# yuhuishi-convect/mojo-bm25

Hardware: AMD Instinct MI355X
Metric: queries/sec + achieved HBM GB/s, 10M-doc CSC index, batch=1024, k=100 (higher is better)
Workload: dtype f32; 1 GPU; c3: 10M docs / 200k vocab, batch=1024, k=100, 8 terms per query; segments=dense, n_docs=10000000, n_terms=200000, nnz=639994696, batch=1024, terms_per_query=8, k=100, tile_docs=2048, parallelism=doc-shard x1, term_lanes=8

## Files before the change

mojo-bm25_amd/csrc/bm25mi_kernels.hip:

```cpp
#include "bm25mi_internal.h"

#include <map>
#include <mutex>
#include <cstdio>
#include <cstdlib>
#include <vector>

namespace bm25mi {

enum Phase { kAll = 0, kSample = 1, kRest = 2 };

constexpr int kJ = 8;
constexpr int kWaves = 4;
constexpr int kGroup = 64;

struct IndexArgs {
  const int64_t* indptr;
  const uint32_t* rel;
  const uint16_t* ldoc;
  const float* val;
  int64_t V, ntiles, n_docs, nnz;
  int64_t doc_offset;
  int32_t nonneg;
  int32_t sparse;
// ... 481 lines not shown
        ++pos;
      }
    }
  }
  zero_acc<S>(acc);
}

template <int S>
__device__ __forceinline__ void emit_rest_slot(float* acc, int64_t tile, int64_t n_docs,
                                               uint64_t theta, uint64_t* __restrict__ slot,
                                               int32_t Cb, int32_t* __restrict__ slot_n,
                                               uint64_t* __restrict__ ovf,
                                               int32_t* __restrict__ ovf_cnt, int32_t Co) {
  constexpr int D = 1 << S;
  float4* a4 = reinterpret_cast<float4*>(acc);
  const uint32_t lane = lane_id();
  const float th = key_score((uint32_t)(theta >> 32));
  const int64_t base = tile << S;
  const int lim = (int)max<int64_t>(-1, min<int64_t>(D, n_docs - base));
  const int tie = (int)max<int64_t>(
      -1, min<int64_t>(D, (int64_t)(0xFFFFFFFFu - (uint32_t)theta) - base + 1));
  int32_t n = 0;
#pragma unroll 1
  for (int j0 = 0; j0 < D / 256; j0 += 2) {
    const float4 f0 = a4[j0 * 64 + lane], f1 = a4[(j0 + 1) * 64 + lane];
    const float fe[8] = {f0.x, f0.y, f0.z, f0.w, f1.x, f1.y, f1.z, f1.w};
    const float mx = fmaxf(fmaxf(fmaxf(fe[0], fe[1]), fmaxf(fe[2], fe[3])),
                           fmaxf(fmaxf(fe[4], fe[5]), fmaxf(fe[6], fe[7])));
    int c = 0;
    if (!(mx < th && lim == D)) {
#pragma unroll
      for (int e = 0; e < 8; ++e) {
        const int d = (int)entry_doc(4 * j0 + e, lane);
        c += (d < lim) & ((fe[e] > th) | ((fe[e] == th) & (d < tie)));
      }
    }
    if (__ballot(c > 0) == 0) continue;
    const uint32_t incl = wave_incl_scan((uint32_t)c);
    const int32_t tot = (int32_t)__builtin_amdgcn_readlane(incl, 63);
    int pos = n + (int)incl - c;
    const int32_t past = max(n, Cb);
    int obase = 0;
    if (n + tot > past) {
      if (lane == 0) obase = atomicAdd(ovf_cnt, n + tot - past);
      obase = __shfl(obase, 0, 64) - past;
    }
#pragma unroll
    for (int e = 0; e < 8; ++e) {
      const int d = (int)entry_doc(4 * j0 + e, lane);
      const bool pass = (d < lim) & ((fe[e] > th) | ((fe[e] == th) & (d < tie)));
      if (pass) {
        const uint64_t key = ((uint64_t)score_key(fe[e]) << 32) |
                             (uint64_t)(0xFFFFFFFFu - (uint32_t)(base + d));
        if (pos < Cb) slot[pos] = key;
        else if (obase + pos < Co) ovf[obase + pos] = key;
        ++pos;
      }
    }
    n += tot;
  }
  if (n > 0 && lane == 0) *slot_n = n;
  zero_acc<S>(acc);
}

constexpr int kCrossCap = 256;
template <int S>
__device__ __forceinline__ void emit_cross(float* acc, const uint16_t* xl, int32_t nx,
                                           int64_t tile, int64_t n_docs, uint64_t theta,
                                           uint64_t* __restrict__ slot, int32_t Cb,
                                           int32_t* __restrict__ slot_n,
                                           uint64_t* __restrict__ ovf,
                                           int32_t* __restrict__ ovf_cnt, int32_t Co) {
  constexpr int D = 1 << S;
  const uint32_t lane = lane_id();
  const float th = key_score((uint32_t)(theta >> 32));
  const int64_t base = tile << S;
  const int lim = (int)max<int64_t>(-1, min<int64_t>(D, n_docs - base));
  const int tie = (int)max<int64_t>(
      -1, min<int64_t>(D, (int64_t)(0xFFFFFFFFu - (uint32_t)theta) - base + 1));
  int32_t n = 0;
  for (int32_t i0 = 0; i0 < nx; i0 += 64) {
    const int32_t i = i0 + (int32_t)lane;
    const uint32_t off = i < nx ? (uint32_t)xl[i] : 0u;
    const int d = (int)(off >> 2);
    const float f = i < nx ? atomicExch(&acc[d], -1.0f) : -1.0f;
    const bool pass = i < nx && f >= 0.f && d < lim && ((f > th) | ((f == th) & (d < tie)));
    const uint64_t m = __ballot(pass);
    if (m == 0ull) continue;
    const int32_t tot = (int32_t)__popcll(m);
    const int pos = n + (int)__builtin_amdgcn_mbcnt_hi((uint32_t)(m >> 32),
                                                     __builtin_amdgcn_mbcnt_lo((uint32_t)m, 0u));
    const int32_t past = max(n, Cb);
    int obase = 0;
    if (n + tot > past) {
      if (lane == 0) obase = atomicAdd(ovf_cnt, n + tot - past);
      obase = __shfl(obase, 0, 64) - past;
    }
    if (pass) {
      const uint64_t key = ((uint64_t)score_key(f) << 32) |
                           (uint64_t)(0xFFFFFFFFu - (uint32_t)(base + d));
      if (pos < Cb) slot[pos] = key;
      else if (obase + pos < Co) ovf[obase + pos] = key;
    }
    n += tot;
  }
  if (n > 0 && lane == 0) *slot_n = n;
  zero_acc<S>(acc);
}

template <int PH>
__device__ __forceinline__ int64_t tile_of(int64_t ti, int P, int G) {
  return PH == kSample ? sample_tile(ti, P, G) : ti;
}
template <int PH>
__device__ __forceinline__ int32_t tile_of32(uint32_t ti, uint32_t P, uint32_t G) {
  return (int32_t)(PH == kSample ? ((ti & ~(G - 1u)) * P) | (ti & (G - 1u)) : ti);
}


struct PostingRsrc {
  __amdgpu_buffer_rsrc_t ldoc, val;
};

__device__ __forceinline__ PostingRsrc posting_rsrc(const IndexArgs& a) {
  PostingRsrc r;
  const int np = (int)(a.nnz + kPostingPad);
  r.ldoc = __builtin_amdgcn_make_buffer_rsrc((void*)a.ldoc, 0, (int)((uint32_t)np * 2u), 0x00020000);
  r.val = __builtin_amdgcn_make_buffer_rsrc((void*)a.val, 0, (int)((uint32_t)np * 4u), 0x00020000);
  return r;
}
typedef uint32_t bm25_v2u __attribute__((ext_vector_type(2)));
__device__ uint32_t bm25_sload_b32(__amdgpu_buffer_rsrc_t r, int vindex, int voffset, int soffset,
                                   int aux) __asm("llvm.amdgcn.struct.ptr.buffer.load.i32");
__device__ bm25_v2u bm25_sload_b64(__amdgpu_buffer_rsrc_t r, int vindex, int voffset, int soffset,
                                   int aux) __asm("llvm.amdgcn.struct.ptr.buffer.load.v2i32");

__device__ __forceinline__ PostingRsrc posting_rsrc_pairs(const IndexArgs& a) {
  PostingRsrc r;
  const int np2 = (int)((a.nnz + kPostingPad) >> 1);
  r.ldoc = __builtin_amdgcn_make_buffer_rsrc((void*)a.ldoc, 4, np2, 0x00020000);
  r.val = __builtin_amdgcn_make_buffer_rsrc((void*)a.val, 8, np2, 0x00020000);
  return r;
}

template <int S, int M, bool POS = false>
__device__ __forceinline__ void best_dense(float* acc, int64_t tile, int64_t n_docs,
                                           uint32_t idoff, uint64_t* __restrict__ out) {
  constexpr int E = (1 << S) / 64;
  const float4* a4 = reinterpret_cast<const float4*>(acc);
  const uint32_t lane = lane_id();
  const int64_t base = tile << S;
  const int lim = (int)min<int64_t>(1 << S, n_docs - base);
  uint32_t bk[M], bd[M];
#pragma unroll
  for (int i = 0; i < M; ++i) {
    bk[i] = 0;
    bd[i] = 0;
  }
  constexpr int per = E / 4 / M;
#pragma unroll
  for (int i = 0; i < M; ++i) {
#pragma unroll 2
    for (int jj = 0; jj < per; ++jj) {
      const int j = i * per + jj;
      const float4 f = a4[j * 64 + lane];
      const float fe[4] = {f.x, f.y, f.z, f.w};
#pragma unroll
      for (int c = 0; c < 4; ++c) {
        const uint32_t key =
            (POS && !(fe[c] > 0.f)) ? 0u : entry_key(fe[c], 4 * j + c, lane, lim);
        if (key > bk[i]) {
          bk[i] = key;
          bd[i] = entry_doc(4 * j + c, lane);
        }
      }
    }
  }
  zero_acc<S>(acc);
#pragma unroll
  for (int i = 0; i < M; ++i) {
    const uint32_t wm = wave_max_u32(bk[i]);
    uint64_t key = 0ull;
    if (wm != 0) {
      const uint32_t doc = 0xFFFFFFFFu - wave_max_u32(bk[i] == wm ? 0xFFFFFFFFu - bd[i] : 0u);
      key = ((uint64_t)wm << 32) | (uint64_t)(0xFFFFFFFFu - (uint32_t)(base + doc) - idoff);
    }
    if (lane_id() == 0) out[i] = key;
  }
}

template <int S, int M>
__device__ __forceinline__ void best_slices_pos(float* acc, int64_t tile, int64_t n_docs,
                                                uint32_t idoff, uint64_t* __restrict__ out) {
  constexpr int per = (1 << S) / 256 / M;
  static_assert(per >= 1, "a slice holds at least one float4 per lane");
  const float4* a4 = reinterpret_cast<const float4*>(acc);
  const uint32_t lane = lane_id();
  const int64_t base = tile << S;
#pragma unroll
  for (int i = 0; i < M; ++i) {
    float m = 0.f;
#pragma unroll
    for (int jj = 0; jj < per; ++jj) {
      const float4 f = a4[(i * per + jj) * 64 + lane];
      m = fmaxf(m, fmaxf(fmaxf(f.x, f.y), fmaxf(f.z, f.w)));
    }
    const uint32_t wm = wave_max_u32(__float_as_uint(m));
    const int64_t last = min<int64_t>(base + (int64_t)(i + 1) * per * 256 - 1, n_docs - 1);
    const uint64_t key = wm == 0u ? 0ull
                         : ((uint64_t)score_key(__uint_as_float(wm)) << 32) |
                               (uint64_t)(0xFFFFFFFFu - (uint32_t)last - idoff);
    if (lane == (uint32_t)i) out[i] = key;
  }
  zero_acc<S>(acc);
}

template <int S>
__device__ __forceinline__ void best1_pos(float* acc, int64_t tile, uint32_t idoff,
                                          uint64_t* __restrict__ out, uint64_t* mirror) {
  constexpr int E4 = (1 << S) / 256;
  float4* a4 = reinterpret_cast<float4*>(acc);
  const uint32_t lane = lane_id();
  float m = 0.f;
#pragma unroll
  for (int j = 0; j < E4; ++j) {
    const float4 f = a4[j * 64 + lane];
    m = fmaxf(m, fmaxf(fmaxf(f.x, f.y), fmaxf(f.z, f.w)));
  }
  const uint32_t wm = wave_max_u32(__float_as_uint(m));
  uint64_t key = 0ull;
  if (wm != 0u) {
    const float fm = __uint_as_float(wm);
    uint32_t bd = 0xFFFFFFFFu;
#pragma unroll
    for (int j = E4 - 1; j >= 0; --j) {
      const float4 f = a4[j * 64 + lane];
      bd = f.w == fm ? entry_doc(4 * j + 3, lane) : bd;
      bd = f.z == fm ? entry_doc(4 * j + 2, lane) : bd;
      bd = f.y == fm ? entry_doc(4 * j + 1, lane) : bd;
      bd = f.x == fm ? entry_doc(4 * j + 0, lane) : bd;
    }
    const uint32_t doc = 0xFFFFFFFFu - wave_max_u32(0xFFFFFFFFu - bd);
    key = ((uint64_t)score_key(fm) << 32) |
          (uint64_t)(0xFFFFFFFFu - (uint32_t)((tile << S) + doc) - idoff);
  }
  zero_acc<S>(acc);
  if (lane == 0) *out = key;
  if (lane == 1 && mirror) *mirror = key;
}
template <int S, int PH>
__global__ __launch_bounds__(64 * kWaves) void score_wave_kernel(
    IndexArgs a, const int32_t* __restrict__ queries, int32_t T, Stage sg,
    const uint64_t* __restrict__ theta, uint64_t* __restrict__ cand, uint64_t* __restrict__ list,
    int32_t* __restrict__ list_cnt, int32_t C) {
  constexpr int D = 1 << S;
  __shared__ __attribute__((aligned(16))) float acc_all[kWaves * D];
  const int wave = uniform((int)(threadIdx.x >> 6));
  float* acc = acc_all + wave * D;
  const int64_t nq = sg.nq_dev ? (int64_t)*sg.nq_dev : (int64_t)sg.nq_host;
  const int P = sg.P;
  const int64_t nt = PH == kSample ? sample_count(a.ntiles, P, sg.G) : a.ntiles;
  const int64_t nitems = nt * nq;
  const int64_t per = (nitems + 7) >> 3;
  const int64_t grp = blockIdx.x & 7;
  const int64_t lo = grp * per;
  const int64_t hi = min(nitems, lo + per);
  const int64_t stride = (int64_t)(gridDim.x >> 3) * kWaves;
  int64_t it = lo + (int64_t)(blockIdx.x >> 3) * kWaves + wave;
  if (it >= hi) return;
  zero_acc<S>(acc);
  for (; it < hi; it += stride) {
    const int64_t ti = it / nq;
    const int64_t qi = it - ti * nq;
    const int64_t q = sg.qmap ? (int64_t)sg.qmap[qi] : qi;
    const int64_t tile = tile_of<PH>(ti, P, sg.G);
    add_item<S>(a, tile, queries + q * T, T, acc);
    float fv[D / 64];
    take_entries<S>(acc, fv);
    if (PH == kRest)
      emit_above<S>(fv, tile, a.n_docs, theta[qi], list + qi * C, list_cnt + qi, C);
    else
      select_top<S>(fv, tile, a.n_docs, PH == kSample ? sg.M : kTileM,
                    PH == kSample ? (uint32_t)a.doc_offset : 0u,
                    sg.cand_out + qi * sg.cstride + ti * (PH == kSample ? sg.M : kTileM));
  }
}
#ifndef BM25_QW
#define BM25_QW 4
#endif
constexpr int kQW = BM25_QW;
#ifndef BM25_FR
#define BM25_FR 10
#endif
#ifndef BM25_FR_S
#define BM25_FR_S 8
#endif

#ifndef BM25_FLAT_WPE
#define BM25_FLAT_WPE 5
#endif

#ifndef BM25_CLAMP
#define BM25_CLAMP 2
#endif

#ifndef BM25_TRACE
#define BM25_TRACE 0
#endif
#if BM25_TRACE
constexpr int kTraceWaves = 1 << 14;
__device__ uint64_t g_bm25_trace[4 * kTraceWaves];
#endif

__device__ __forceinline__ uint32_t scan64(uint32_t x) {
  x += (uint32_t)__builtin_amdgcn_update_dpp(0, (int)x, 0x111, 0xF, 0xF, true);
  x += (uint32_t)__builtin_amdgcn_update_dpp(0, (int)x, 0x112, 0xF, 0xF, true);
  x += (uint32_t)__builtin_amdgcn_update_dpp(0, (int)x, 0x114, 0xF, 0xF, true);
  x += (uint32_t)__builtin_amdgcn_update_dpp(0, (int)x, 0x118, 0xF, 0xF, true);
  x += (uint32_t)__builtin_amdgcn_update_dpp(0, (int)x, 0x142, 0xA, 0xF, false);
  x += (uint32_t)__builtin_amdgcn_update_dpp(0, (int)x, 0x143, 0xC, 0xF, false);
  return x;
}

struct FlatCur {
  int32_t rit, end, b, q, qb, bw;
};

struct FlatDesc {
  uint32_t ip, r0, r1;
  uint32_t aux;
};

__device__ __forceinline__ float f16_bits_to_float(uint16_t h) {
  _Float16 x;
  __builtin_memcpy(&x, &h, 2);
  return (float)x;
}

constexpr uint32_t kRowNewTile = 1u << 17;
constexpr uint32_t kRowParity = 1u << 24;
constexpr uint32_t kRowDead = 1u << 25;
__device__ __forceinline__ uint32_t row_lo(uint32_t w) { return w & 1u; }
__device__ __forceinline__ uint32_t row_n0(uint32_t w) { return (w >> 1) & 0xFFu; }
__device__ __forceinline__ uint32_t row_n1(uint32_t w) { return (w >> 9) & 0xFFu; }
__device__ __forceinline__ uint32_t row_tile(uint32_t w) { return (w >> 18) & 0x3Fu; }

struct FlatTab {
  uint32_t base;
  uint32_t w;
  uint32_t last;
};

struct FlatCtx {
  int32_t q, b;
  uint64_t th;
};

constexpr uint32_t kNoTile = 0xFFFFFFFFu;
__device__ __forceinline__ uint32_t kth_set_bit16(uint32_t m, uint32_t k) {
  uint32_t pos = 0u;
  uint32_t c = (uint32_t)__popc(m & 0xFFu);
  if (k >= c) { k -= c; pos = 8u; m >>= 8; }
  c = (uint32_t)__popc(m & 0xFu);
  if (k >= c) { k -= c; pos += 4u; m >>= 4; }
  c = (uint32_t)__popc(m & 3u);
  if (k >= c) { k -= c; pos += 2u; m >>= 2; }
  if (k >= (m & 1u)) pos += 1u;
  return pos;
}
template <int TL, bool RW = false>
__device__ __forceinline__ FlatTab flat_chunk(uint32_t sb, uint32_t sl, uint32_t incl,
                                              uint32_t excl, uint32_t total, uint32_t j0,
                                              uint32_t prev, uint32_t par) {
  const uint32_t lane = lane_id();
  const uint32_t j = j0 + lane;
  int pos = 0;
#pragma unroll
  for (int step = 32; step >= 1; step >>= 1) {
    const uint32_t x = (uint32_t)__shfl((int)incl, pos + step - 1, 64);
    if (x <= j) pos += step;
  }
  const uint32_t e = (uint32_t)__shfl((int)excl, pos, 64);
  const uint32_t b = (uint32_t)__shfl((int)sb, pos, 64);
  const uint32_t lw = (uint32_t)__shfl((int)sl, pos, 64);
  const uint32_t l = RW ? (lw & 0xFFFFu) : lw;
  const bool in = j < total;
  FlatTab t;
  uint32_t k = j - e;
  if constexpr (RW) {
    if ((lw >> 16) != 0xFFFFu) k = kth_set_bit16(lw >> 16, k);
  }
  t.base = (in && l != 0u) ? ((b & ~1u) + 128u * k) * 2u : 0u;
  const uint32_t rlo = k == 0u ? (b & 1u) : 0u;
  const uint32_t rhi = min(128u, (b & 1u) + l - 128u * k);
  const uint32_t masks = (in && l != 0u) ? (rlo | ((((rhi + 1u) >> 1) - rlo) << 1) | ((rhi >> 1) << 9))
                                         : 0u;
  const uint32_t tile = (uint32_t)pos >> TL;
  uint32_t tp = (uint32_t)__shfl_up((int)tile, 1, 64);
  if (lane == 0u) tp = prev;
  const uint32_t top1 = masks != 0u ? (((rhi + 1u) >> 1) - 1u) : 0u;
  t.w = masks | ((in && tile != tp) ? kRowNewTile : 0u) | (tile << 18) | (par ? kRowParity : 0u) |
        (top1 << 26);
  t.last = lane_u32(tile, 63);
  return t;
}

__host__ __device__ inline int flat_tl(int64_t T) {
  return T <= 8 ? 3 : (T <= 16 ? 4 : (T <= 32 ? 5 : 6));
}

template <int S, int PH, int SM, bool SP, int TL, bool RW = false>
__global__ __launch_bounds__(64) __attribute__((amdgpu_waves_per_eu(BM25_FLAT_WPE, BM25_FLAT_WPE))) void score_flat_kernel(
    IndexArgs a, const int32_t* __restrict__ queries, int32_t T, int32_t P, int32_t G,
    int32_t nq_host, const int32_t* __restrict__ nq_dev, const int32_t* __restrict__ qmap,
    const uint64_t* __restrict__ theta, uint64_t* __restrict__ cand, int64_t cstride,
    uint64_t* __restrict__ list, int32_t* __restrict__ list_cnt, int32_t C,
    int32_t* __restrict__ wctr, int32_t claim_ch, int32_t claim_m,
    const uint64_t* __restrict__ skeys, int64_t sstride, int32_t BW, uint64_t* mirror,
    int32_t* __restrict__ stats, int32_t* __restrict__ slot_cnt,
    const uint32_t* __restrict__ sub, const int32_t* __restrict__ sub_ipb) {
  constexpr int D = 1 << S;
  constexpr bool kSplit = PH == kRest && SM == kSplitM;
  constexpr int kFR = PH == kSample ? BM25_FR_S : BM25_FR;
  constexpr uint32_t TT = 1u << TL;
  constexpr uint32_t kTileMask = (64u >> TL) - 1u;
  __shared__ __attribute__((aligned(16))) float acc[D + 64];
  constexpr bool kCross = PH == kRest && SM == kLargeM;
  __shared__ uint16_t xl[kCross ? kCrossCap : 1];
  const uint32_t lane = lane_id();
  const uint32_t trash = ((uint32_t)D + lane) * 4u;
  const int32_t nq = (PH == kAll && nq_dev) ? uniform(*nq_dev) : nq_host;
  const int32_t nt = PH == kSample ? (int32_t)sample_count(a.ntiles, P, G) : (int32_t)a.ntiles;
  const int32_t nb = (nt + BW - 1) / BW;
  const int32_t ipb = kSplit ? uniform(*sub_ipb) : nq;
  const int64_t nitems = (int64_t)nb * ipb;
  const int64_t per = (nitems + 7) >> 3;
  const int grp = (int)(blockIdx.x & 7);
  const uint32_t lo = (uint32_t)(grp * per);
  const int32_t ngi = (int32_t)max<int64_t>(0, min<int64_t>(nitems, lo + per) - lo);
  if (ngi == 0) return;
  const int32_t cm = (int32_t)(blockIdx.x >> 3) % claim_m;
  int32_t* ctr = wctr + (grp * kClaimM + cm) * kCtrStride;
  auto finish = [&]() {
    const int32_t g8 = (int32_t)(gridDim.x >> 3);
    const int32_t sharers = g8 / claim_m + (cm < g8 % claim_m ? 1 : 0);
    int32_t old = 0;
    if (lane == 0) old = atomicAdd(ctr + kDoneOff, 1);
    if (uniform(old) == sharers - 1 && lane == 0) {
      ctr[0] = 0;
      ctr[kDoneOff] = 0;
    }
  };
#if BM25_CLAMP == 2
  const PostingRsrc pr = posting_rsrc_pairs(a);
#else
  const PostingRsrc pr = posting_rsrc(a);
#endif
#if BM25_TRACE
  const uint64_t tr_t0 = wall_clock64();
  uint32_t tr_items = 0, tr_rows = 0;
#endif
  const uint32_t lt = lane & (TT - 1u), li = lane >> TL;
  const int64_t nbp = (a.ntiles + 7) >> 3;

  auto dec = [&](FlatCur& c, uint32_t it) {
    const uint32_t band = it / (uint32_t)ipb;
    const uint32_t e = uniform((int)sub[it - band * (uint32_t)ipb]);
    c.q = (int32_t)(e & 0xFFFFFu);
    c.qb = c.q;
    c.b = (int32_t)(band * (uint32_t)BW + ((e >> 20) & 63u));
    c.bw = min((int32_t)(e >> 26), nt - c.b);
  };
  auto claim = [&]() -> int32_t {
    int32_t v = 0;
    if (lane == 0) v = atomicAdd(ctr, 1);
    return v;
  };
  int32_t pending = claim();
  auto batch_row = [&](int32_t q) -> int32_t {
    return (PH == kAll && qmap) ? uniform(qmap[q]) : q;
  };
  auto next = [&](FlatCur c) -> FlatCur {
    if (c.rit >= ngi) return c;
    if (c.rit + 1 < c.end) {
      ++c.rit;
      if constexpr (kSplit) {
        dec(c, lo + (uint32_t)c.rit);
        return c;
      }
      if (++c.q == nq) {
        c.q = 0;
        c.b += BW;
        c.bw = min(BW, nt - c.b);
      }
      c.qb = batch_row(c.q);
      return c;
    }
    const int64_t bb = ((int64_t)uniform(pending) * claim_m + cm) * claim_ch;
    if (bb >= ngi) {
      c.rit = c.end = ngi;
      return c;
    }
    pending = claim();
    FlatCur n;
    n.rit = (int32_t)bb;
    n.end = (int32_t)min<int64_t>(ngi, bb + claim_ch);
    const uint32_t it = lo + (uint32_t)bb;
    if constexpr (kSplit) {
      dec(n, it);
      return n;
    }
    const uint32_t band = it / (uint32_t)nq;
    n.q = (int32_t)(it - band * (uint32_t)nq);
    n.qb = batch_row(n.q);
    n.b = (int32_t)band * BW;
    n.bw = min(BW, nt - n.b);
    return n;
  };
  auto terms_of = [&](const FlatCur& c) -> int32_t {
    return queries[(int64_t)c.qb * T + (int)min(lt, (uint32_t)(T - 1))];
  };
  static_assert(!RW || (PH == kRest && TL == 3 && SM != kLargeM), "row words: 8-lane REST only");
  constexpr bool kBits = RW;
  const bool skipping = PH == kRest && skeys != nullptr && G == kSampleGroup &&
                        !(kBits && a.tskip != nullptr);
  const uint32_t lgG = (uint32_t)__builtin_ctz((unsigned)G), lgP = (uint32_t)__builtin_ctz((unsigned)P);
  auto load_bdesc = [&](const FlatCur& c, int32_t tm) -> FlatDesc {
    FlatDesc d;
    const int32_t term = tm;
    const bool ok = (int)lt < T && (int)li < c.bw && term >= 0 && term < a.V;
    const int64_t tt = ok ? term : 0;
    const int64_t tile = ok ? (int64_t)tile_of32<PH>((uint32_t)(c.b + li), (uint32_t)P,
                                                      (uint32_t)G)
                            : 0;
    if constexpr (SP) {
      const uint64_t e = a.seg[ok ? ((int64_t)c.qb * nbp + (tile >> 3)) * (8 * TT) + lt * 8 + (tile & 7)
                                  : a.seg_zero];
      d.ip = 0u;
      d.r0 = (uint32_t)e;
      d.r1 = (uint32_t)e + (uint32_t)(e >> 32);
    } else {
      const uint32_t* r = a.rel + tt * (a.ntiles + 1) + tile;
      d.ip = (uint32_t)a.indptr[tt];
      d.r0 = r[0];
      d.r1 = *(ok ? r + 1 : r);
    }
    d.aux = 0u;
    if (kBits && a.tskip != nullptr) {
      const uint32_t t32 = (uint32_t)c.b + li;
      if ((int)li < c.bw)
        d.aux = a.tskip[((int64_t)c.q * a.tskip_stride + t32) * 8 + lt];
    } else if (skipping) {
      const uint32_t t32 = (uint32_t)tile;
      const int64_t si = (int64_t)(((t32 >> (lgG + lgP)) << lgG) | (t32 & (uint32_t)(G - 1)));
      d.aux = reinterpret_cast<const uint32_t*>(skeys)[2 * ((int64_t)c.q * sstride +
                                                              min<int64_t>(si, sstride - 1)) + 1];
    }
    return d;
  };
  auto th_positive = [&](uint64_t th) -> bool {
    return (uint32_t)(th >> 32) > score_key(0.f);
  };

  uint32_t nbound = 0;
  constexpr bool kCountPost = PH == kRest && SM == 2;
  uint32_t npost = 0;
  uint32_t ndrop = 0, ndpost = 0;
  uint32_t nrdrop = 0, nrpost = 0;
  uint32_t iSb = 0, iSl = 0, iIncl = 0, iExcl = 0;
  uint32_t iTotal = 0, iR = 0, iJ0 = 0, iPrev = kNoTile, iCur = 0;
  int32_t ctxV = 0, iPar = 0;
  FlatCur nx, nx2;
  FlatDesc dN;
  uint64_t thN = 0ull;
  int32_t tmN2 = 0;
  auto enter_item = [&]() {
#if BM25_TRACE
    ++tr_items;
#endif
    const bool th_pos = PH == kRest && th_positive(thN);
    const uint32_t t32 = (uint32_t)nx.b + li;
    const bool smp = skipping && ((t32 >> lgG) & (uint32_t)(P - 1)) == 0u;
    bool skip = smp && th_pos && dN.aux < (uint32_t)(thN >> 32);
    if constexpr (PH == kRest) {
      if (kBits && a.tskip != nullptr) {
        const bool drop = dN.aux == 0u;
        if constexpr (kCountPost) {
          const bool cut = seg_sum_u32<TL>(drop ? 1u : 0u) == TT;
          const uint32_t sl = dN.r1 - dN.r0;
          const uint32_t tp = seg_sum_u32<TL>(sl);
          const bool cnt = cut && !skip && lt == 0u && (int)li < nx.bw;
          nbound += (uint32_t)__popcll(__ballot(cnt));
          npost += wave_sum_u32(cnt ? tp : 0u);
          const bool dcnt = drop && !cut && !skip && sl != 0u;
          ndrop += (uint32_t)__popcll(__ballot(dcnt));
          ndpost += wave_sum_u32(dcnt ? sl : 0u);
          const uint32_t b1 = (dN.ip + dN.r0) & 1u;
          const uint32_t nf = sl == 0u ? 0u : (b1 + sl + 127u) >> 7;
          const bool rcnt = !drop && !skip && dN.aux != 0xFFFFu;
          uint32_t rr = 0u, rp = 0u;
#pragma unroll
          for (uint32_t r = 0; r < 16u; ++r) {
            if (rcnt && r < nf && ((dN.aux >> r) & 1u) == 0u) {
              ++rr;
              rp += min(128u, b1 + sl - 128u * r) - (r == 0u ? b1 : 0u);
            }
          }
          nrdrop += wave_sum_u32(rr);
          nrpost += wave_sum_u32(rp);
        }
        skip = skip || drop;
      }
    }
    iSb = dN.ip + dN.r0;
    iSl = skip ? 0u : dN.r1 - dN.r0;
    uint32_t nr = iSl == 0u ? 0u : ((iSb & 1u) + iSl + 127u) >> 7;
    if constexpr (kBits) {
      const uint32_t rw = a.tskip != nullptr ? dN.aux : 0xFFFFu;
      if (rw != 0xFFFFu) nr = (uint32_t)__popc(rw & ~(0xFFFFFFFFu << min(nr, 16u)));
      iSl |= rw << 16;
    }
    if ((PH == kAll || (PH == kRest && !th_pos)) && lt == 0u && (int)li < nx.bw)
      nr = max(nr, 1u);
    if constexpr (PH == kSample) {
      const uint32_t tr = seg_sum_u32<TL>(nr);
      if (lt == 0u && (int)li < nx.bw && tr == 0u) {
        uint64_t* out = cand + (int64_t)nx.q * cstride + (int64_t)(nx.b + (int32_t)li) * SM;
#pragma unroll
        for (int i = 0; i < SM; ++i) out[i] = 0ull;
        if (SM == 1 && mirror) mirror[out - cand] = 0ull;
      }
    }
    iIncl = scan64(nr);
    iExcl = iIncl - nr;
    iTotal = lane_u32(iIncl, 63);
    uint32_t R = max(iTotal, (uint32_t)kFR);
    if ((R & 63u) != 0u && (R & 63u) < (uint32_t)kFR) R += (uint32_t)kFR - (R & 63u);
    iR = R;
    iJ0 = 0;
    iPrev = kNoTile;
    {
      const int32_t c4 = (int32_t)lane - 4 * iPar;
      ctxV = c4 == 0 ? nx.q : c4 == 1 ? nx.b : c4 == 2 ? (int32_t)(uint32_t)thN
           : c4 == 3 ? (int32_t)(uint32_t)(thN >> 32) : ctxV;
    }
    iCur = (uint32_t)iPar;
    iPar ^= 1;
    FlatCur nx3 = next(nx2);
    dN = load_bdesc(nx2, tmN2);
    thN = PH == kRest ? theta[nx2.q] : 0ull;
    tmN2 = terms_of(nx3);
    nx = nx2;
    nx2 = nx3;
  };

  FlatCur c0;
  c0.rit = -1;
  c0.end = 0;
  c0.b = c0.q = c0.qb = 0;
  c0.bw = 1;
  nx = next(c0);
  if (nx.rit >= ngi) {
    finish();
    return;
  }
  dN = load_bdesc(nx, terms_of(nx));
  thN = PH == kRest ? theta[nx.q] : 0ull;
  nx2 = next(nx);
  tmN2 = terms_of(nx2);
  for (int j = 0; j < D / 256; ++j)
    reinterpret_cast<float4*>(acc)[j * 64 + lane] = make_float4(0.f, 0.f, 0.f, 0.f);
  acc[D + lane] = -__builtin_inff();

  bool items_left = true;
  FlatTab tI;
  uint32_t nI = 0, il = 0;
  auto next_chunk = [&]() {
    if (iJ0 + 64u < iR) {
      iJ0 += 64u;
      iPrev = tI.last;
    } else if (items_left && nx.rit < ngi) {
      enter_item();
    } else {
      items_left = false;
      tI.base = 0u;
      tI.w = kRowDead;
      nI = 0x7FFFFFFFu;
      il = 0;
      return;
    }
    tI = flat_chunk<TL, kBits>(iSb, iSl, iIncl, iExcl, iTotal, iJ0, iPrev, iCur);
    nI = min(64u, iR - iJ0);
    il = 0;
  };
  enter_item();
  tI = flat_chunk<TL, kBits>(iSb, iSl, iIncl, iExcl, iTotal, 0u, iPrev, iCur);
  nI = min(64u, iR);
  il = 0;

  uint32_t ldR[kFR], wR[kFR];
  float v0R[kFR], v1R[kFR];
  auto issue = [&](int s) {
    if (il == nI) next_chunk();
    const uint32_t base = lane_u32(tI.base, (int)il);
    wR[s] = lane_u32(tI.w, (int)il);
#if BM25_CLAMP == 2
    const int li2 = (int)min(lane, wR[s] >> 26);
    ldR[s] = bm25_sload_b32(pr.ldoc, li2, 0, (int)base, 0);
    const bm25_v2u v = bm25_sload_b64(pr.val, li2, 0, (int)(base * 2u), 0);
    v0R[s] = __uint_as_float(v[0]);
    v1R[s] = __uint_as_float(v[1]);
#else
#if BM25_CLAMP
    const uint32_t wv = wR[s];
    const uint32_t top = max(row_lo(wv) + row_n0(wv), row_n1(wv));
    const uint32_t t4 = (top > 0u ? top - 1u : 0u) * 4u;
    const uint32_t lo4 = min(lane * 4u, t4), lo8 = min(lane * 8u, 2u * t4);
#else
    const uint32_t lo4 = lane * 4u, lo8 = lane * 8u;
#endif
    ldR[s] = __builtin_amdgcn_raw_buffer_load_b32(pr.ldoc, (int)lo4, (int)base, 0);
    const auto v = __builtin_amdgcn_raw_buffer_load_b64(pr.val, (int)lo8, (int)(base * 2u), 0);
    v0R[s] = __uint_as_float((uint32_t)v[0]);
    v1R[s] = __uint_as_float((uint32_t)v[1]);
#endif
    ++il;
  };
#pragma unroll
  for (int s = 0; s < kFR; ++s) issue(s);

  FlatCtx ctxE{0, 0, 0ull};
  uint32_t curTi = kNoTile;
  float hmax = 0.f;
  bool done = false;
  float thS = 0.f;
  int32_t ncross = 0;

  auto epilogue = [&]() {
    const int32_t ti = ctxE.b + (int32_t)curTi;
    const int64_t tile = tile_of32<PH>((uint32_t)ti, (uint32_t)P, (uint32_t)G);
    if constexpr (kCross) {
      const int64_t si = (int64_t)ctxE.q * a.ntiles + tile;
      if (ncross == 0)
        zero_acc<S>(acc);
      else if (ncross <= kCrossCap)
        emit_cross<S>(acc, xl, ncross, tile, a.n_docs, ctxE.th, cand + si * cstride,
                      (int32_t)cstride, slot_cnt + si, list + (int64_t)ctxE.q * C,
                      list_cnt + ctxE.q, C);
      else
        emit_rest_slot<S>(acc, tile, a.n_docs, ctxE.th, cand + si * cstride, (int32_t)cstride,
                          slot_cnt + si, list + (int64_t)ctxE.q * C, list_cnt + ctxE.q, C);
    } else if constexpr (PH == kRest) {
      const bool flagged = a.nonneg && th_positive(ctxE.th);
      if (flagged && __ballot(hmax >= key_score((uint32_t)(ctxE.th >> 32))) == 0) {
        zero_acc<S>(acc);
      } else {
        emit_rest<S>(acc, tile, a.n_docs, ctxE.th, list + (int64_t)ctxE.q * C,
                     list_cnt + ctxE.q, C);
      }
      hmax = 0.f;
    } else if constexpr (PH == kAll) {
      select_top_lds<S>(acc, tile, a.n_docs, kTileM, cand + (int64_t)ctxE.q * cstride + tile * kTileM);
    } else {
      uint64_t* out = cand + (int64_t)ctxE.q * cstride + (int64_t)ti * SM;
      if constexpr (SM == 1) {
        if (a.nonneg) {
          const uint32_t wm = wave_max_u32(__float_as_uint(hmax));
          const uint32_t last = (uint32_t)min<int64_t>((tile << S) + D - 1, a.n_docs - 1);
          const uint64_t key = wm == 0u ? 0ull
                               : ((uint64_t)score_key(__uint_as_float(wm)) << 32) |
                                     (uint64_t)(0xFFFFFFFFu - last - (uint32_t)a.doc_offset);
          zero_acc<S>(acc);
          if (lane == 0) *out = key;
          if (lane == 1 && mirror) mirror[out - cand] = key;
          hmax = 0.f;
        } else {
          best1_pos<S>(acc, tile, (uint32_t)a.doc_offset, out, mirror ? mirror + (out - cand) : nullptr);
        }
      } else if (SM == kLargeM || a.nonneg) {
        best_slices_pos<S, SM>(acc, tile, a.n_docs, (uint32_t)a.doc_offset, out);
      } else {
        best_dense<S, SM, true>(acc, tile, a.n_docs, (uint32_t)a.doc_offset, out);
      }
    }
  };

  uint32_t sc0, sc1, wC;
  float ac0, ac1, xc0, xc1;
  auto lds_at = [&](uint32_t off) -> float& {
    return *reinterpret_cast<float*>(reinterpret_cast<char*>(acc) + off);
  };
  auto prepare = [&](int s) {
    wC = wR[s];
    const bool m0 = lane - row_lo(wC) < row_n0(wC), m1 = lane < row_n1(wC);
    sc0 = m0 ? (ldR[s] & 0xFFFFu) : trash;
    sc1 = m1 ? (ldR[s] >> 16) : trash;
    ac0 = v0R[s];
    ac1 = v1R[s];
    xc0 = lds_at(sc0);
    xc1 = lds_at(sc1);
  };
  prepare(0);

  auto step = [&](int s) {
    issue(s);
    if (wC & kRowNewTile) {
      if (curTi != kNoTile) epilogue();
      curTi = row_tile(wC) & kTileMask;
      const int32_t pPar = (wC & kRowParity) ? 1 : 0;
      ctxE.q = __builtin_amdgcn_readlane(ctxV, 4 * pPar);
      ctxE.b = __builtin_amdgcn_readlane(ctxV, 4 * pPar + 1);
      ctxE.th = ((uint64_t)(uint32_t)__builtin_amdgcn_readlane(ctxV, 4 * pPar + 3) << 32) |
                (uint32_t)__builtin_amdgcn_readlane(ctxV, 4 * pPar + 2);
      xc0 = sc0 == trash ? xc0 : 0.f;
      xc1 = sc1 == trash ? xc1 : 0.f;
      if constexpr (kCross) {
        thS = key_score((uint32_t)(ctxE.th >> 32));
        ncross = th_positive(ctxE.th) ? 0 : kCrossCap + 1;
      }
    }
    const float y0 = xc0 + ac0, y1 = xc1 + ac1;
    lds_at(sc0) = y0;
    lds_at(sc1) = y1;
    if constexpr (kCross) {
      const uint64_t m0 = __ballot(y0 >= thS);
      const uint64_t m1 = __ballot(y1 >= thS);
      if ((m0 | m1) != 0ull) {
        const int32_t n0 = (int32_t)__popcll(m0), n1 = (int32_t)__popcll(m1);
        if (ncross + n0 + n1 <= kCrossCap) {
          const uint32_t b0 = __builtin_amdgcn_mbcnt_hi((uint32_t)(m0 >> 32),
                                                        __builtin_amdgcn_mbcnt_lo((uint32_t)m0, 0u));
          const uint32_t b1 = __builtin_amdgcn_mbcnt_hi((uint32_t)(m1 >> 32),
                                                        __builtin_amdgcn_mbcnt_lo((uint32_t)m1, 0u));
          if ((m0 >> lane) & 1ull) xl[ncross + (int32_t)b0] = (uint16_t)sc0;
          if ((m1 >> lane) & 1ull) xl[ncross + n0 + (int32_t)b1] = (uint16_t)sc1;
        }
        ncross += n0 + n1;
      }
    } else if (PH == kRest || (PH == kSample && SM == 1)) {
      hmax = fmaxf(hmax, fmaxf(y0, y1));
    }
    done = (wC & kRowDead) != 0u;
    prepare((s + 1) % kFR);
  };

  while (!done) {
#pragma unroll
    for (int s = 0; s < kFR; ++s) step(s);
#if BM25_TRACE
    tr_rows += kFR;
#endif
  }
#if BM25_TRACE
  if (PH == kRest && lane == 0 && blockIdx.x < kTraceWaves) {
    uint64_t* tr = g_bm25_trace + 4 * blockIdx.x;
    tr[0] = tr_t0;
    tr[1] = wall_clock64();
    tr[2] = tr_items;
    tr[3] = tr_rows;
  }
#endif
  if (curTi != kNoTile) epilogue();
  if (kCountPost && stats != nullptr) {
    const uint32_t nb = nbound;
    if (lane == 0 && nb != 0u) atomicAdd(stats, (int32_t)nb);
    const uint32_t np = npost;
    if (lane == 0 && np != 0u)
      atomicAdd(reinterpret_cast<unsigned long long*>(stats + 1), (unsigned long long)np);
    const uint32_t nd = ndrop;
    if (lane == 0 && nd != 0u) atomicAdd(stats + 3, (int32_t)nd);
    const uint32_t ndp = ndpost;
    if (lane == 0 && ndp != 0u)
      atomicAdd(reinterpret_cast<unsigned long long*>(stats + 5), (unsigned long long)ndp);
    const uint32_t nrd = nrdrop;
    if (lane == 0 && nrd != 0u) atomicAdd(stats + 4, (int32_t)nrd);
    const uint32_t nrp = nrpost;
    if (lane == 0 && nrp != 0u)
      atomicAdd(reinterpret_cast<unsigned long long*>(stats + 7), (unsigned long long)nrp);
  }
  finish();
}

constexpr int kRescoreNT = 256;

__device__ __forceinline__ void bitonic_sort_desc(uint64_t* keys, int n) {
  for (int size = 2; size <= n; size <<= 1) {
    for (int stride = size >> 1; stride > 0; stride >>= 1) {
      const int ls = __builtin_ctz((unsigned)stride);
      for (int i = threadIdx.x; i < (n >> 1); i += blockDim.x) {
        const int lo = ((i >> ls) << (ls + 1)) + (i & (stride - 1));
        const int hi = lo + stride;
        const bool desc = (lo & size) == 0;
        const uint64_t x = keys[lo], y = keys[hi];
        if ((x < y) == desc) {
          keys[lo] = y;
          keys[hi] = x;
        }
      }
      __syncthreads();
    }
  }
}

template <int S>
__device__ void rescore_tile(const IndexArgs& a, const int32_t* __restrict__ queries, int32_t T,
                             int32_t k, int64_t q, int64_t tile, uint64_t* out, float* acc,
                             uint64_t* keys) {
  constexpr int D = 1 << S;
  if (threadIdx.x < 64) {
    zero_acc<S>(acc);
    add_item<S>(a, tile, queries + q * T, T, acc);
  }
  __syncthreads();
  for (int i = threadIdx.x; i < D; i += blockDim.x) {
    const int64_t doc = (tile << S) + i;
    keys[i] = doc < a.n_docs ? make_key(acc[i], (uint32_t)doc) : 0ull;
  }
  __syncthreads();
  bitonic_sort_desc(keys, D);
  for (int i = threadIdx.x; i < k; i += blockDim.x) out[i] = i < D ? keys[i] : 0ull;
}

template <int S>
__global__ __launch_bounds__(kRescoreNT) void rescore_kernel(IndexArgs a,
                                                             const int32_t* __restrict__ queries,
                                                             int32_t T, int32_t k, int64_t maxflag,
                                                             Stage sg, Workspace ws) {
  constexpr int D = 1 << S;
  __shared__ __attribute__((aligned(16))) float acc[D];
  __shared__ uint64_t keys[D];
  __shared__ int32_t s_item;
  const int32_t n_items = ws.counters[0];
  for (;;) {
    __syncthreads();
    if (threadIdx.x == 0) s_item = atomicAdd(&ws.counters[1], 1);
    __syncthreads();
    const int32_t it = s_item;
    if (it >= n_items) break;
    const int32_t code = ws.queue[it];
    const int64_t qi = code / maxflag;
    const int64_t q = sg.qmap ? (int64_t)sg.qmap[qi] : qi;
    const int64_t tile = sample_tile(ws.flag_tiles[code], sg.P, sg.G);
    rescore_tile<S>(a, queries, T, k, q, tile, ws.cand2 + (int64_t)code * k, acc, keys);
  }
}

template <int S>
__global__ __launch_bounds__(64) void scores_dense_kernel(IndexArgs a,
                                                          const int32_t* __restrict__ query,
                                                          int32_t T, float* __restrict__ out) {
  constexpr int D = 1 << S, E = D / 64;
  __shared__ __attribute__((aligned(16))) float acc[D];
  const int64_t tile = blockIdx.x;
  zero_acc<S>(acc);
  add_item<S>(a, tile, query, T, acc);
  float fv[E];
  take_entries<S>(acc, fv);
  const int64_t base = tile << S;
  const uint32_t lane = lane_id();
  if (base + D <= a.n_docs) {
#pragma unroll
    for (int j = 0; j < E / 4; ++j)
      *reinterpret_cast<float4*>(out + base + entry_doc(4 * j, lane)) =
          make_float4(fv[4 * j], fv[4 * j + 1], fv[4 * j + 2], fv[4 * j + 3]);
  } else {
#pragma unroll
    for (int e = 0; e < E; ++e)
      if (base + entry_doc(e, lane) < a.n_docs) out[base + entry_doc(e, lane)] = fv[e];
  }
}

template <int S, bool WT = false>
__global__ __launch_bounds__(64) void scores_batch_kernel(IndexArgs a,
                                                          const int32_t* __restrict__ queries,
                                                          int32_t T, int64_t stride,
                                                          float* __restrict__ out,
                                                          const float* __restrict__ weights) {
  constexpr int D = 1 << S, E = D / 64;
  __shared__ __attribute__((aligned(16))) float acc[D];
  const int64_t tile = blockIdx.x, g = blockIdx.y;
  zero_acc<S>(acc);
  add_item<S, WT>(a, tile, queries + g * T, T, acc, WT ? weights + g * T : nullptr);
  float fv[E];
  take_entries<S>(acc, fv);
  float* row = out + g * stride + (tile << S);
  const uint32_t lane = lane_id();
#pragma unroll
  for (int j = 0; j < E / 4; ++j)
    *reinterpret_cast<float4*>(row + entry_doc(4 * j, lane)) =
        make_float4(fv[4 * j], fv[4 * j + 1], fv[4 * j + 2], fv[4 * j + 3]);
}

__global__ __launch_bounds__(256) void build_tables_kernel(
    const int64_t* __restrict__ indptr, const int32_t* __restrict__ indices, int64_t V,
    int64_t n_docs, int S, int64_t ntiles, uint32_t* __restrict__ rel,
    uint16_t* __restrict__ ldoc, int32_t* __restrict__ err) {
  const int lane = lane_id();
  const int64_t waves = (int64_t)gridDim.x * (blockDim.x >> 6);
  const uint32_t mask = (1u << S) - 1u;
  for (int64_t t = (int64_t)blockIdx.x * (blockDim.x >> 6) + (threadIdx.x >> 6); t < V;
       t += waves) {
    const int64_t a0 = indptr[t], a1 = indptr[t + 1];
    const int64_t df = a1 - a0;
    uint32_t* row = rel + t * (ntiles + 1);
    const bool heavy = df * 4 >= ntiles;
    for (int64_t p = a0 + lane; p < a1; p += 64) {
      const int32_t d = indices[p];
      const int32_t dp = p > a0 ? indices[p - 1] : -1;
      const bool ok = d >= 0 && (int64_t)d < n_docs && d > dp;
      if (!ok) atomicOr(err, 1);
      ldoc[p] = (uint16_t)(((uint32_t)d & mask) << 2);
      if (heavy && ok) {
        const int64_t tp = dp >= 0 ? ((int64_t)dp >> S) : -1;
        const int64_t tc = (int64_t)d >> S;
        for (int64_t j = tp + 1; j <= tc; ++j) row[j] = (uint32_t)(p - a0);
      }
    }
    if (heavy) {
      int64_t last = -1;
      if (df > 0) {
        const int32_t dl = indices[a1 - 1];
        last = (dl >= 0 && (int64_t)dl < n_docs) ? ((int64_t)dl >> S) : ntiles - 1;
      }
      for (int64_t j = last + 1 + lane; j <= ntiles; j += 64) row[j] = (uint32_t)df;
    } else {
      for (int64_t j = lane; j <= ntiles; j += 64) {
        const int64_t target = j << S;
        int64_t lo = 0, hi = df;
        while (lo < hi) {
          const int64_t mid = (lo + hi) >> 1;
          if ((int64_t)indices[a0 + mid] < target) lo = mid + 1;
          else hi = mid;
        }
        row[j] = (uint32_t)lo;
      }
    }
  }
}

__global__ __launch_bounds__(256) void build_bmax_kernel(const int64_t* __restrict__ indptr,
                                                         const uint32_t* __restrict__ rel,
                                                         const float* __restrict__ val, int64_t V,
                                                         int64_t ntiles,
                                                         uint16_t* __restrict__ bmax) {
  const int64_t bs = bmax_stride(ntiles);
  for (int64_t t = blockIdx.x; t < V; t += gridDim.x) {
    const int64_t ip = indptr[t];
    const uint32_t* r = rel + t * (ntiles + 1);
    for (int64_t j = ntiles + threadIdx.x; j < bs; j += blockDim.x) bmax[t * bs + j] = 0;
    for (int64_t j = threadIdx.x; j < ntiles; j += blockDim.x) {
      float m = 0.f;
      for (int64_t p = ip + r[j]; p < ip + r[j + 1]; ++p) m = fmaxf(m, val[p]);
      _Float16 h = (_Float16)m;
      uint16_t u;
      __builtin_memcpy(&u, &h, 2);
      if ((float)h > m) --u;
      bmax[t * bs + j] = u;
    }
  }
}

__global__ __launch_bounds__(256) void build_tmask_kernel(const int64_t* __restrict__ indptr,
                                                          const uint32_t* __restrict__ rel,
                                                          const uint16_t* __restrict__ ldoc,
                                                          int64_t V, int64_t ntiles, int S,
                                                          uint32_t* __restrict__ tmask) {
  const int64_t bs = bmax_stride(ntiles);
  for (int64_t t = blockIdx.x; t < V; t += gridDim.x) {
    const int64_t ip = indptr[t];
    const uint32_t* r = rel + t * (ntiles + 1);
    for (int64_t j = ntiles + threadIdx.x; j < bs; j += blockDim.x) tmask[t * bs + j] = 0u;
    for (int64_t j = threadIdx.x; j < ntiles; j += blockDim.x) {
      uint32_t m = 0u;
      for (int64_t p = ip + r[j]; p < ip + r[j + 1]; ++p) m |= 1u << ((uint32_t)ldoc[p] >> (S - 3));
      tmask[t * bs + j] = m;
    }
  }
}

__global__ __launch_bounds__(256) void heavy_terms_kernel(const int64_t* __restrict__ indptr,
                                                          const uint32_t* __restrict__ rel,
                                                          int64_t V, int64_t ntiles,
                                                          int32_t* __restrict__ heavy) {
  for (int64_t t = blockIdx.x; t < V; t += gridDim.x) {
    const int64_t ip = indptr[t];
    const uint32_t* r = rel + t * (ntiles + 1);
    int any = 0;
    for (int64_t j = threadIdx.x; j < ntiles; j += blockDim.x) {
      const uint32_t l = r[j + 1] - r[j];
      any |= (((uint32_t)(ip + r[j]) & 1u) + l + 127u) >> 7 >= 2u;
    }
    any = __syncthreads_or(any);
    if (threadIdx.x == 0) heavy[t] = any;
  }
}

__global__ __launch_bounds__(256) void build_rowmask_kernel(const int64_t* __restrict__ indptr,
                                                            const uint32_t* __restrict__ rel,
                                                            const uint16_t* __restrict__ ldoc,
                                                            const int32_t* __restrict__ hterm,
                                                            int64_t H, int64_t ntiles, int S,
                                                            uint32_t* __restrict__ rowmask) {
  for (int64_t h = blockIdx.x; h < H; h += gridDim.x) {
    const int64_t t = hterm[h];
    const int64_t ip = indptr[t];
    const uint32_t* r = rel + t * (ntiles + 1);
    for (int64_t j = threadIdx.x; j < ntiles; j += blockDim.x) {
      uint32_t* out = rowmask + (h * ntiles + j) * kRowEntries;
      const int64_t b = ip + r[j], e = ip + r[j + 1];
      const int64_t b0 = b & ~(int64_t)1;
      const bool wide = e > b && ((e - 1 - b0) >> 7) >= kRowEntries;
      for (int i = 0; i < kRowEntries; ++i) out[i] = wide ? 0xFFFFFFFFu : 0u;
      if (wide) continue;
      int64_t cur = 0;
      uint32_t m = 0u;
      for (int64_t p = b; p < e; ++p) {
        const int64_t row = (p - b0) >> 7;
        if (row != cur) {
          out[cur] = m;
          m = 0u;
          cur = row;
        }
        m |= 1u << ((uint32_t)ldoc[p] >> (S - 3));
      }
      if (e > b) out[cur] = m;
    }
  }
}

constexpr int kSkipNT = 256;
constexpr int kSkipTerms = 8;
inline int skip_npt(int64_t ntiles) {
  const int64_t bs = bmax_stride(ntiles);
  return bs >= 4 * kSkipNT ? 4 : (bs >= 2 * kSkipNT ? 2 : 1);
}
constexpr uint32_t kSkipBias = 0x80000000u - 1048472u;
template <int N> struct alignas(2 * N) SkipB { uint16_t v[N]; };
template <int N> struct alignas(4 * N) SkipM { uint32_t v[N]; };
struct alignas(16) SkipW { uint16_t v[kSkipTerms]; };
template <int N>
__global__ __launch_bounds__(kSkipNT) void tile_skip_kernel(
    const uint16_t* __restrict__ bmax, const uint32_t* __restrict__ tmask, int64_t V,
    int64_t ntiles, const int32_t* __restrict__ queries, int32_t T, int64_t Q,
    const uint64_t* __restrict__ theta, uint16_t* __restrict__ tskip, int32_t seg,
    const int32_t* __restrict__ hslot, const uint32_t* __restrict__ rowmask) {
  const int64_t bs = bmax_stride(ntiles);
  const int64_t nch = (bs + kSkipNT * N - 1) / (kSkipNT * N);
  for (int64_t it = blockIdx.x; it < Q * nch; it += gridDim.x) {
    const int64_t q = it / nch;
    const int64_t t0 = ((it - q * nch) * kSkipNT + threadIdx.x) * N;
    if (t0 >= bs) continue;
    const uint32_t thk = (uint32_t)(theta[q] >> 32);
    SkipW* dst = reinterpret_cast<SkipW*>(tskip) + q * bs + t0;
    SkipW all;
#pragma unroll
// ... 2444 lines not shown
```

Measured before the change: 542,400 queries/s.

## Hoist chunk refill and tile-change handling out of the unrolled ring loop

```diff
diff --git a/mojo-bm25_amd/csrc/bm25mi_kernels.hip b/mojo-bm25_amd/csrc/bm25mi_kernels.hip
--- a/mojo-bm25_amd/csrc/bm25mi_kernels.hip
+++ b/mojo-bm25_amd/csrc/bm25mi_kernels.hip
@@ -807,6 +807,10 @@
 
 #ifndef BM25_CLAMP
 #define BM25_CLAMP 2
+#endif
+
+#ifndef BM25_FLAT_LOOP
+#define BM25_FLAT_LOOP 1
 #endif
 
 #ifndef BM25_TRACE
@@ -966,6 +970,15 @@
   uint32_t tr_items = 0, tr_rows = 0;
 #endif
   const uint32_t lt = lane & (TT - 1u), li = lane >> TL;
+#if BM25_FLAT_LOOP
+  auto item_lane = [&]() -> uint32_t {
+    uint32_t l = lane;
+    asm volatile("" : "+v"(l));
+    return l;
+  };
+#else
+  auto item_lane = [&]() -> uint32_t { return lane; };
+#endif
   const int64_t nbp = (a.ntiles + 7) >> 3;
 
   auto dec = [&](FlatCur& c, uint32_t it) {
@@ -1023,6 +1036,7 @@
     return n;
   };
   auto terms_of = [&](const FlatCur& c) -> int32_t {
+    const uint32_t lt = item_lane() & (TT - 1u);
     return queries[(int64_t)c.qb * T + (int)min(lt, (uint32_t)(T - 1))];
   };
   static_assert(!RW || (PH == kRest && TL == 3 && SM != kLargeM), "row words: 8-lane REST only");
@@ -1032,6 +1046,8 @@
   const uint32_t lgG = (uint32_t)__builtin_ctz((unsigned)G), lgP = (uint32_t)__builtin_ctz((unsigned)P);
   auto load_bdesc = [&](const FlatCur& c, int32_t tm) -> FlatDesc {
     FlatDesc d;
+    const uint32_t il_ = item_lane();
+    const uint32_t lt = il_ & (TT - 1u), li = il_ >> TL;
     const int32_t term = tm;
     const bool ok = (int)lt < T && (int)li < c.bw && term >= 0 && term < a.V;
     const int64_t tt = ok ? term : 0;
@@ -1206,7 +1222,9 @@
   uint32_t ldR[kFR], wR[kFR];
   float v0R[kFR], v1R[kFR];
   auto issue = [&](int s) {
+#if !BM25_FLAT_LOOP
     if (il == nI) next_chunk();
+#endif
     const uint32_t base = lane_u32(tI.base, (int)il);
     wR[s] = lane_u32(tI.w, (int)il);
 #if BM25_CLAMP == 2
@@ -1307,23 +1325,29 @@
   };
   prepare(0);
 
+  auto tile_change = [&]() {
+    if (curTi != kNoTile) epilogue();
+    curTi = row_tile(wC) & kTileMask;
+    const int32_t pPar = (wC & kRowParity) ? 1 : 0;
+    ctxE.q = __builtin_amdgcn_readlane(ctxV, 4 * pPar);
+    ctxE.b = __builtin_amdgcn_readlane(ctxV, 4 * pPar + 1);
+    ctxE.th = ((uint64_t)(uint32_t)__builtin_amdgcn_readlane(ctxV, 4 * pPar + 3) << 32) |
+              (uint32_t)__builtin_amdgcn_readlane(ctxV, 4 * pPar + 2);
+    xc0 = sc0 == trash ? xc0 : 0.f;
+    xc1 = sc1 == trash ? xc1 : 0.f;
+    if constexpr (kCross) {
+      thS = key_score((uint32_t)(ctxE.th >> 32));
+      ncross = th_positive(ctxE.th) ? 0 : kCrossCap + 1;
+    }
+  };
   auto step = [&](int s) {
+#if BM25_TRACE
+    ++tr_rows;
+#endif
     issue(s);
-    if (wC & kRowNewTile) {
-      if (curTi != kNoTile) epilogue();
-      curTi = row_tile(wC) & kTileMask;
-      const int32_t pPar = (wC & kRowParity) ? 1 : 0;
-      ctxE.q = __builtin_amdgcn_readlane(ctxV, 4 * pPar);
-      ctxE.b = __builtin_amdgcn_readlane(ctxV, 4 * pPar + 1);
-      ctxE.th = ((uint64_t)(uint32_t)__builtin_amdgcn_readlane(ctxV, 4 * pPar + 3) << 32) |
-                (uint32_t)__builtin_amdgcn_readlane(ctxV, 4 * pPar + 2);
-      xc0 = sc0 == trash ? xc0 : 0.f;
-      xc1 = sc1 == trash ? xc1 : 0.f;
-      if constexpr (kCross) {
-        thS = key_score((uint32_t)(ctxE.th >> 32));
-        ncross = th_positive(ctxE.th) ? 0 : kCrossCap + 1;
-      }
-    }
+#if !BM25_FLAT_LOOP
+    if (wC & kRowNewTile) tile_change();
+#endif
     const float y0 = xc0 + ac0, y1 = xc1 + ac1;
     lds_at(sc0) = y0;
     lds_at(sc1) = y1;
@@ -1349,13 +1373,58 @@
     prepare((s + 1) % kFR);
   };
 
+#if BM25_FLAT_LOOP
+  static_assert(kFR <= 16, "ring slots: the switch below has 16 cases");
+  auto pending_event = [&]() -> bool {
+    return il == nI || (wC & kRowNewTile) != 0u;
+  };
+#define BM25_FLAT_SLOT(N)                                   \
+  case N:                                                   \
+    if constexpr ((N) < kFR) {                              \
+      step((N) < kFR ? (N) : 0);                            \
+      if constexpr ((N) + 1 < kFR) {                        \
+        if (pending_event()) {                              \
+          resume = (N) + 1;                                 \
+          break;                                            \
+        }                                                   \
+      } else {                                              \
+        resume = 0;                                         \
+        break;                                              \
+      }                                                     \
+    }                                                       \
+    [[fallthrough]];
+  int resume = 0;
   while (!done) {
+    if (il == nI) next_chunk();
+    if (wC & kRowNewTile) tile_change();
+    switch (resume) {
+      BM25_FLAT_SLOT(0)
+      BM25_FLAT_SLOT(1)
+      BM25_FLAT_SLOT(2)
+      BM25_FLAT_SLOT(3)
+      BM25_FLAT_SLOT(4)
+      BM25_FLAT_SLOT(5)
+      BM25_FLAT_SLOT(6)
+      BM25_FLAT_SLOT(7)
+      BM25_FLAT_SLOT(8)
+      BM25_FLAT_SLOT(9)
+      BM25_FLAT_SLOT(10)
+      BM25_FLAT_SLOT(11)
+      BM25_FLAT_SLOT(12)
+      BM25_FLAT_SLOT(13)
+      BM25_FLAT_SLOT(14)
+      BM25_FLAT_SLOT(15)
+      default:
+        resume = 0;
+    }
+  }
+#undef BM25_FLAT_SLOT
+#else
+  while (!done) {
 #pragma unroll
     for (int s = 0; s < kFR; ++s) step(s);
-#if BM25_TRACE
-    tr_rows += kFR;
+  }
 #endif
-  }
 #if BM25_TRACE
   if (PH == kRest && lane == 0 && blockIdx.x < kTraceWaves) {
     uint64_t* tr = g_bm25_trace + 4 * blockIdx.x;
```

New measurement: 388,100 queries/s. 28.4% lower.
